# ashrafgt/k8s-gpu-hpa

Measured on AMD Instinct MI355X. Metric: p50_scrape_to_hpa_scale_latency, lower is better.
Workload: dtype bf16; 1 GPU; model=mi355x-exporter + mfma-bf16-gemm load, load=gemm_bf16 4096^3 duty-cycled, hpa=target 5, min 1, max 8 (reference rule semantics), parallelism=replicas1, gpus_exported=0, final_replicas=8, tick_aligned_steps=30, stale_steps=0

## Files before the change

### __graft_entry__.py

```python

import subprocess
import sys
from pathlib import Path

ROOT = Path(__file__).resolve().parent


def build() -> None:
    subprocess.run(
        ["make", "-C", str(ROOT / "native"), "all", "-j4",
         f"PYTHON={sys.executable}"],
        check=True,
    )
    sys.path.insert(0, str(ROOT))
    import mi355x_gpu_hpa
    import mi355x_gpu_hpa.loadgen as lg

    assert lg.available(), "libmi355x_loadgen.so missing after build"
    from mi355x_gpu_hpa.control import scraper

    assert scraper.native_available(), "libmi355x_scrape.so missing after build"
    from mi355x_gpu_hpa.control import promql

    assert promql.native_available(), (
        "_mi355x_promql extension missing after build (needs Python.h)")


def smoke() -> None:
    sys.path.insert(0, str(ROOT))
    import numpy as np
    import torch

    from mi355x_gpu_hpa import loadgen as lg

    assert torch.cuda.is_available(), "smoke() needs a GPU"
    assert lg.device_count() >= 1, lg.LoadgenError("no HIP device visible")

    rng = np.random.default_rng(0)
    a = rng.standard_normal(4096, dtype=np.float32)
    b = rng.standard_normal(4096, dtype=np.float32)
    np.testing.assert_array_equal(lg.vector_add(a, b), a + b)

    m, n, k = 128, 128, 64
    A = rng.uniform(-1, 1, (m, k)).astype(np.float32)
    Bt = rng.uniform(-1, 1, (n, k)).astype(np.float32)
    got = lg.gemm_bf16(A, Bt)
    ref = (
        torch.from_numpy(A).bfloat16().float()
        @ torch.from_numpy(Bt).bfloat16().float().T
    ).numpy()
    np.testing.assert_allclose(got, ref, rtol=2e-2, atol=1e-2)

    m, n, k = 256, 256, 128
    A = rng.uniform(-1, 1, (m, k)).astype(np.float32)
    Bt = rng.uniform(-1, 1, (n, k)).astype(np.float32)
    c, aq, btq = lg.gemm_fp8(A, Bt)
    ref8 = (aq.astype(np.float64) @ btq.astype(np.float64).T).astype(np.float32)
    np.testing.assert_allclose(c, ref8, rtol=2e-3, atol=2e-3 * np.sqrt(k))

    m, n, k = 256, 256, 256
    A = rng.uniform(-1, 1, (m, k)).astype(np.float32)
    Bt = rng.uniform(-1, 1, (n, k)).astype(np.float32)
    c, aq, btq = lg.gemm_mxfp4(A, Bt)
    ref4 = aq.astype(np.float64) @ btq.astype(np.float64).T
    np.testing.assert_allclose(
        c, ref4, rtol=2e-3,
        atol=2e-3 * np.sqrt(k) * np.abs(aq).max() * np.abs(btq).max())

    from mi355x_gpu_hpa.exporter import native_exporter_smoke

    native_exporter_smoke()
    print("smoke OK: vectorAdd + bf16/fp8/mxfp4 MFMA GEMM numerics + exporter sample")
```

### mi355x_gpu_hpa/control/__init__.py

```python
from .adapter import Adapter, AdapterError, DiscoveredMetric, discover
from .hpa import (
    HpaSpec,
    HpaState,
    MetricTarget,
    desired_replicas,
    desired_replicas_multi,
    reconcile,
    reconcile_multi,
)
from .loop import (
    REFERENCE_RULE_EXPR,
    REFERENCE_RULE_NAME,
    ControlLoop,
    LoopResult,
    RecordingRule,
    synth_pod_labels,
)
from .promql import PromQLError, Sample, evaluate, evaluate_scalar
from .scraper import Scraper, ScrapeTarget, parse_prometheus_text

__all__ = [
    "Adapter", "AdapterError", "DiscoveredMetric", "discover",
    "HpaSpec", "HpaState", "MetricTarget", "desired_replicas",
    "desired_replicas_multi", "reconcile", "reconcile_multi",
    "ControlLoop", "LoopResult", "RecordingRule", "synth_pod_labels",
    "REFERENCE_RULE_EXPR", "REFERENCE_RULE_NAME",
    "PromQLError", "Sample", "evaluate", "evaluate_scalar",
    "Scraper", "ScrapeTarget", "parse_prometheus_text",
]
```

### mi355x_gpu_hpa/control/adapter.py

```python

from __future__ import annotations

import re
from dataclasses import dataclass, field
from typing import Dict, List, Optional, Set, Tuple

from .promql import PromQLError, Sample, evaluate

RESOURCE_LABELS: Dict[str, Tuple[str, str, str]] = {
    "namespace": ("namespaces", "", "Namespace"),
    "pod": ("pods", "", "Pod"),
    "node": ("nodes", "", "Node"),
    "service": ("services", "", "Service"),
    "deployment": ("deployments", "apps", "Deployment"),
    "statefulset": ("statefulsets", "apps", "StatefulSet"),
    "daemonset": ("daemonsets", "apps", "DaemonSet"),
    "replicaset": ("replicasets", "apps", "ReplicaSet"),
    "job": ("jobs", "batch", "Job"),
    "ingress": ("ingresses", "networking.k8s.io", "Ingress"),
}

_PLURAL_TO_SINGULAR = {v[0]: k for k, v in RESOURCE_LABELS.items()}


class AdapterError(ValueError):
    pass


@dataclass
class DiscoveredMetric:

    metric: str
    series: str
    is_counter: bool
    resources: Set[str] = field(default_factory=set)


def _discoverable(s: Sample) -> bool:
    if not s.name or s.name.startswith("container_"):
        return False
    return bool(s.labels.get("namespace"))


def _metric_name(series: str) -> Tuple[str, bool]:
    m = re.match(r"^(.*)_seconds_total$", series)
    if m:
        return m.group(1), True
    m = re.match(r"^(.*)_total$", series)
    if m:
        return m.group(1), True
    return series, False


def discover(samples: List[Sample]) -> Dict[str, DiscoveredMetric]:
    out: Dict[str, DiscoveredMetric] = {}
    for s in samples:
        if not _discoverable(s):
            continue
        metric, is_counter = _metric_name(s.name)
        d = out.get(metric)
        if d is None:
            d = DiscoveredMetric(metric=metric, series=s.name,
                                 is_counter=is_counter)
            out[metric] = d
        for label, value in s.labels.items():
            if value and label in RESOURCE_LABELS:
                d.resources.add(label)
    return out


class Adapter:

    def __init__(self, samples: Optional[List[Sample]] = None):
        self._samples: List[Sample] = list(samples or [])

    def update(self, samples: List[Sample]) -> None:
        self._samples = list(samples)


    def api_resource_list(self) -> dict:
        resources = []
        for d in sorted(discover(self._samples).values(),
                        key=lambda d: d.metric):
            for label in sorted(d.resources):
                plural, group, _kind = RESOURCE_LABELS[label]
                qualified = plural if not group else f"{plural}.{group}"
                resources.append({
                    "name": f"{qualified}/{d.metric}",
                    "singularName": "",
                    "namespaced": label != "namespace",
                    "kind": "MetricValueList",
                    "verbs": ["get"],
                })
        return {
            "kind": "APIResourceList",
            "apiVersion": "v1",
            "groupVersion": "custom.metrics.k8s.io/v1beta1",
            "resources": resources,
        }

    def metric_names(self) -> Set[str]:
        return {r["name"] for r in self.api_resource_list()["resources"]}


    def get_object_metric(self, namespace: str, resource: str,
                          object_name: str, metric: str) -> dict:
        singular = _PLURAL_TO_SINGULAR.get(resource)
        if singular is None:
            raise AdapterError(f"unknown resource {resource!r}")
        for val in (namespace, object_name):
            if not re.fullmatch(r"[A-Za-z0-9._-]{1,253}", val or ""):
                raise AdapterError(f"invalid object name {val!r}")
        discovered = discover(self._samples)
        d = discovered.get(metric)
        if d is None or singular not in d.resources:
            raise AdapterError(
                f"metric {metric!r} not served for resource {resource!r}")
        if d.is_counter:
            raise AdapterError(
                f"metric {metric!r} uses a rate() query; an instant store "
                "has no range data (counters are out of this stack's path)")
        expr = (f'sum({d.series}{{namespace="{namespace}",'
                f'{singular}="{object_name}"}}) by ({singular})')
        try:
            vec = evaluate(expr, self._samples)
        except PromQLError as e:
            raise AdapterError(f"query failed: {e}") from e
        if not vec:
            raise AdapterError(
                f"no samples for {metric!r} on {resource}/{object_name} "
                f"in namespace {namespace!r}")
        plural, group, kind = RESOURCE_LABELS[singular]
        api_version = f"{group}/v1" if group else "v1"
        return {
            "kind": "MetricValueList",
            "apiVersion": "custom.metrics.k8s.io/v1beta1",
            "items": [{
                "describedObject": {
                    "kind": kind,
                    "namespace": namespace,
                    "name": object_name,
                    "apiVersion": api_version,
                },
                "metricName": metric,
                "value": vec[0].value,
            }],
        }

    def get_object_metric_value(self, namespace: str, resource: str,
                                object_name: str, metric: str
                                ) -> Optional[float]:
        try:
            resp = self.get_object_metric(namespace, resource,
                                          object_name, metric)
        except AdapterError:
            return None
        return float(resp["items"][0]["value"])
```

### mi355x_gpu_hpa/control/hpa.py

```python

from __future__ import annotations

import math
from dataclasses import dataclass, field
from typing import List, Optional, Tuple


@dataclass
class HpaSpec:
    min_replicas: int = 1
    max_replicas: int = 3
    target_value: float = 5.0
    tolerance: float = 0.1
    downscale_stabilization_s: float = 300.0
    scale_up_pods: int = 0
    scale_up_period_s: float = 15.0
    scale_down_pods: int = 0
    scale_down_period_s: float = 15.0


@dataclass
class HpaState:
    current_replicas: int = 1
    recommendations: List[Tuple[float, int]] = field(default_factory=list)
    scaleup_window: Tuple[Optional[float], Optional[int]] = (None, None)
    scaledown_window: Tuple[Optional[float], Optional[int]] = (None, None)


def desired_replicas(
    spec: HpaSpec, current_replicas: int, metric_value: Optional[float]
) -> int:
    clamp = lambda r: max(spec.min_replicas, min(spec.max_replicas, r))
    if metric_value is None:
        return clamp(current_replicas)
    if spec.target_value <= 0:
        raise ValueError("target_value must be positive")
    ratio = metric_value / spec.target_value
    if abs(ratio - 1.0) <= spec.tolerance:
        return clamp(current_replicas)
    return clamp(math.ceil(ratio * current_replicas))


@dataclass
class MetricTarget:

    name: str
    target_value: float


def desired_replicas_multi(
    spec: HpaSpec,
    metrics: List[MetricTarget],
    current_replicas: int,
    values: dict,
) -> int:
    desired = spec.min_replicas
    any_value = False
    for m in metrics:
        v = values.get(m.name)
        if v is None:
            d = current_replicas
        else:
            any_value = True
            one = HpaSpec(
                min_replicas=spec.min_replicas,
                max_replicas=spec.max_replicas,
                target_value=m.target_value,
                tolerance=spec.tolerance,
            )
            d = desired_replicas(one, current_replicas, v)
        desired = max(desired, d)
    if not any_value:
        return current_replicas
    return desired


def reconcile(
    spec: HpaSpec, state: HpaState, metric_value: Optional[float], now_s: float
) -> int:
    desired = desired_replicas(spec, state.current_replicas, metric_value)
    return _stabilize(spec, state, desired, now_s)


def reconcile_multi(
    spec: HpaSpec, state: HpaState, metrics: List[MetricTarget],
    values: dict, now_s: float
) -> int:
    desired = desired_replicas_multi(spec, metrics, state.current_replicas, values)
    return _stabilize(spec, state, desired, now_s)


def _stabilize(spec: HpaSpec, state: HpaState, desired: int, now_s: float) -> int:
    state.recommendations.append((now_s, desired))
    cutoff = now_s - spec.downscale_stabilization_s
    state.recommendations = [(t, d) for (t, d) in state.recommendations if t >= cutoff]

    stabilized = max(d for (_, d) in state.recommendations)
    new = stabilized
    if spec.scale_up_pods > 0 and new > state.current_replicas:
        base_t, base_r = state.scaleup_window
        if base_t is None or now_s - base_t >= spec.scale_up_period_s:
            base_t, base_r = now_s, state.current_replicas
        new = min(new, base_r + spec.scale_up_pods)
        state.scaleup_window = (base_t, base_r)
    if spec.scale_down_pods > 0 and new < state.current_replicas:
        base_t, base_r = state.scaledown_window
        if base_t is None or now_s - base_t >= spec.scale_down_period_s:
            base_t, base_r = now_s, state.current_replicas
        new = max(new, base_r - spec.scale_down_pods)
        state.scaledown_window = (base_t, base_r)
    new = max(spec.min_replicas, min(spec.max_replicas, new))
    state.current_replicas = new
    return new
```

### mi355x_gpu_hpa/control/scraper.py

```python

from __future__ import annotations

import ctypes
import os
import re
import time
import urllib.parse
import urllib.request
from array import array
from dataclasses import dataclass
from typing import Dict, List, Optional

from .. import NATIVE_BUILD
from .promql import Sample

SCRAPE_LIB = NATIVE_BUILD / "libmi355x_scrape.so"
NATIVE_ENV = "MI355X_SCRAPE_NATIVE"

_LINE_RE = re.compile(
    r"^(?P<name>[a-zA-Z_:][a-zA-Z0-9_:]*)"
    r"(?:\{(?P<labels>[^}]*)\})?\s+"
    r"(?P<value>[+-]?(?:\d+\.?\d*(?:[eE][+-]?\d+)?|Inf|NaN))"
    r"(?:\s+(?P<ts>-?\d+))?$"
)
_LABEL_RE = re.compile(r'([a-zA-Z_][a-zA-Z0-9_]*)="((?:[^"\\]|\\.)*)"')


def parse_prometheus_text(text: str) -> List[Sample]:
    out: List[Sample] = []
    for line in text.splitlines():
        line = line.strip()
        if not line or line.startswith("#"):
            continue
        m = _LINE_RE.match(line)
        if not m:
            continue
        labels = {}
        if m.group("labels"):
            for lm in _LABEL_RE.finditer(m.group("labels")):
                labels[lm.group(1)] = lm.group(2).replace('\\"', '"').replace(
                    "\\\\", "\\"
                )
        v = m.group("value")
        value = float("inf") if v == "Inf" else float("nan") if v == "NaN" else float(v)
        out.append(Sample(m.group("name"), labels, value))
    return out



_OK, _DEFER, _ERR_UNSUPPORTED = 0, 1, -5


class _Result(ctypes.Structure):
    _fields_ = [
        ("n_samples", ctypes.c_int32),
        ("n_strings", ctypes.c_int32),
        ("arena_len", ctypes.c_int32),
        ("body_len", ctypes.c_int32),
        ("http_status", ctypes.c_int32),
        ("connects", ctypes.c_int32),
        ("values", ctypes.c_void_p),
        ("label_counts", ctypes.c_void_p),
        ("arena", ctypes.c_void_p),
        ("body", ctypes.c_void_p),
    ]


_lib = None
_lib_tried = False


def _load_native():
    global _lib, _lib_tried
    if not _lib_tried:
        _lib_tried = True
        try:
            lib = ctypes.CDLL(str(SCRAPE_LIB))
        except OSError:
            return None
        lib.mi355x_scrape_open.restype = ctypes.c_void_p
        lib.mi355x_scrape_open.argtypes = [
            ctypes.c_char_p, ctypes.c_int, ctypes.c_char_p, ctypes.c_char_p,
            ctypes.c_double]
        lib.mi355x_scrape_close.restype = None
        lib.mi355x_scrape_close.argtypes = [ctypes.c_void_p]
        lib.mi355x_scrape_fetch.argtypes = [
            ctypes.c_void_p, ctypes.POINTER(_Result)]
        lib.mi355x_scrape_parse.argtypes = [
            ctypes.c_void_p, ctypes.c_char_p, ctypes.c_int,
            ctypes.POINTER(_Result)]
        _lib = lib
    return _lib


def native_available() -> bool:
    return _load_native() is not None


def _native_enabled_by_env() -> bool:
    return os.environ.get(NATIVE_ENV, "1").strip().lower() not in (
        "0", "false", "off", "no")


def _samples_from_result(res: _Result) -> List[Sample]:
    n = res.n_samples
    if n == 0:
        return []
    strs = ctypes.string_at(res.arena, res.arena_len).decode().split("\n")
    if len(strs) != res.n_strings + 1:
        raise ValueError("scrape library returned an inconsistent arena")
    counts = array("i")
    counts.frombytes(ctypes.string_at(res.label_counts, 4 * n))
    values = array("d")
    values.frombytes(ctypes.string_at(res.values, 8 * n))
    out: List[Sample] = []
    i = 0
    for k, v in zip(counts, values):
        j = i + 1 + 2 * k
        out.append(Sample(strs[i],
                          dict(zip(strs[i + 1:j:2], strs[i + 2:j:2])), v))
        i = j
    return out


class NativeScrapeError(OSError):

    def __init__(self, code: int, http_status: int = 0):
        super().__init__(f"native scrape failed: code {code}"
                         + (f", HTTP {http_status}" if http_status else ""))
        self.code = code
        self.http_status = http_status


class NativeClient:

    def __init__(self, host: str, port: int, path: str = "/metrics",
                 host_header: str = "", timeout_s: float = 2.0):
        lib = _load_native()
        if lib is None:
            raise OSError(f"{SCRAPE_LIB} missing; run `make -C native exporter`")
        self._lib = lib
        self._res = _Result()
        self._h = lib.mi355x_scrape_open(
            host.encode(), port, path.encode(), host_header.encode(),
            float(timeout_s))
        if not self._h:
            raise ValueError(f"bad scrape target {host!r}:{port}")

    @property
    def connects(self) -> int:
        return self._res.connects

    def _finish(self, rc: int) -> List[Sample]:
        res = self._res
        if rc == _OK:
            return _samples_from_result(res)
        if rc == _DEFER:
            return parse_prometheus_text(
                ctypes.string_at(res.body, res.body_len).decode())
        raise NativeScrapeError(rc, res.http_status)

    def fetch(self) -> List[Sample]:
        return self._finish(
            self._lib.mi355x_scrape_fetch(self._h, ctypes.byref(self._res)))

    def parse(self, data: bytes) -> List[Sample]:
        return self._finish(self._lib.mi355x_scrape_parse(
            self._h, data, len(data), ctypes.byref(self._res)))

    def close(self) -> None:
        if self._h:
            self._lib.mi355x_scrape_close(self._h)
            self._h = None

    def __del__(self):
        try:
            self.close()
        except Exception:
            pass


_parse_client: Optional[NativeClient] = None


def native_parse_prometheus_text(text: str) -> List[Sample]:
    global _parse_client
    if _parse_client is None:
        _parse_client = NativeClient("127.0.0.1", 1)
    return _parse_client.parse(text.encode())


def _native_target(url: str):
    try:
        u = urllib.parse.urlsplit(url)
        port = u.port
    except ValueError:
        return None
    if u.scheme != "http" or not u.hostname or u.username or u.password \
            or u.fragment:
        return None
    path = (u.path or "/") + ("?" + u.query if u.query else "")
    if any(c <= " " or c > "~" for c in path + u.netloc):
        return None
    return u.hostname, port or 80, path, u.netloc


@dataclass
class ScrapeTarget:
    url: str
    node: str = "node0"
    extra_labels: Optional[Dict[str, str]] = None


class Scraper:

    def __init__(self, targets: List[ScrapeTarget], timeout_s: float = 2.0,
                 native: Optional[bool] = None):
        self.targets = targets
        self.timeout_s = timeout_s
        self.last: Dict[str, List[Sample]] = {}
        self.last_scrape_duration_s: float = 0.0
        if native is None:
            native = _native_enabled_by_env()
        self.native = bool(native) and native_available()
        self._clients: Dict[str, Optional[tuple]] = {}

    def _client(self, url: str) -> Optional[NativeClient]:
        entry = self._clients.get(url, False)
        if entry and entry[0] != self.timeout_s:
            entry[1].close()
            entry = False
        if entry is False:
            spec = _native_target(url)
            entry = None
            if spec is not None:
                host, port, path, host_header = spec
                entry = (self.timeout_s, NativeClient(
                    host, port, path, host_header, self.timeout_s))
            self._clients[url] = entry
        return entry[1] if entry else None

    def _fetch_python(self, url: str) -> List[Sample]:
        with urllib.request.urlopen(url, timeout=self.timeout_s) as r:
            text = r.read().decode()
        return parse_prometheus_text(text)

    def _fetch(self, url: str) -> List[Sample]:
        client = self._client(url) if self.native else None
        if client is None:
            return self._fetch_python(url)
        try:
            return client.fetch()
        except NativeScrapeError as e:
            if e.code != _ERR_UNSUPPORTED:
                raise
            client.close()
            self._clients[url] = None
            return self._fetch_python(url)

    def close(self) -> None:
        for entry in self._clients.values():
            if entry:
                entry[1].close()
        self._clients.clear()

    def scrape_once(self) -> List[Sample]:
        t0 = time.monotonic()
        merged: List[Sample] = []
        for t in self.targets:
            try:
                samples = self._fetch(t.url)
            except Exception:
                merged.extend(self.last.get(t.url, []))
                continue
            for s in samples:
                s.labels.setdefault("node", t.node)
                if t.extra_labels:
                    for k, v in t.extra_labels.items():
                        s.labels.setdefault(k, v)
            self.last[t.url] = samples
            merged.extend(samples)
        self.last_scrape_duration_s = time.monotonic() - t0
        return merged
```

Baseline: 92.14 us.

## Move scrape relabelling, object-metric lookup and HPA reconcile into a native extension

Adds a C++ Python extension that handles the per-cycle control path natively: HTTP scrape plus parse with node and extra-label relabelling, the adapter's object-metric lookup through the native PromQL evaluator, and the HPA desired-replica and stabilization logic. Each Python entry point tries the native path first and falls back to the Python code when the extension returns DEFER. The goal is to cut Python interpreter and object-churn overhead on each scrape-to-scale cycle. In exchange there is a lot of duplicated logic that must match the Python semantics exactly, along with a string cache whose contents are cleared once it fills.

Result: faster. 58.63 us, median of 6 (-36.4%).

```diff
diff --git a/__graft_entry__.py b/__graft_entry__.py
--- a/__graft_entry__.py
+++ b/__graft_entry__.py
@@ -24,6 +24,10 @@
 
     assert promql.native_available(), (
         "_mi355x_promql extension missing after build (needs Python.h)")
+    from mi355x_gpu_hpa.control import native_cycle
+
+    assert native_cycle.native_cycle_available(), (
+        "_mi355x_control extension missing after build (needs Python.h)")
 
 
 def smoke() -> None:
diff --git a/mi355x_gpu_hpa/control/__init__.py b/mi355x_gpu_hpa/control/__init__.py
--- a/mi355x_gpu_hpa/control/__init__.py
+++ b/mi355x_gpu_hpa/control/__init__.py
@@ -16,6 +16,11 @@
     RecordingRule,
     synth_pod_labels,
 )
+from .native_cycle import (
+    native_cycle_active,
+    native_cycle_counters,
+    use_native_cycle,
+)
 from .promql import PromQLError, Sample, evaluate, evaluate_scalar
 from .scraper import Scraper, ScrapeTarget, parse_prometheus_text
 
@@ -25,6 +30,7 @@
     "desired_replicas_multi", "reconcile", "reconcile_multi",
     "ControlLoop", "LoopResult", "RecordingRule", "synth_pod_labels",
     "REFERENCE_RULE_EXPR", "REFERENCE_RULE_NAME",
+    "native_cycle_active", "native_cycle_counters", "use_native_cycle",
     "PromQLError", "Sample", "evaluate", "evaluate_scalar",
     "Scraper", "ScrapeTarget", "parse_prometheus_text",
 ]
diff --git a/mi355x_gpu_hpa/control/adapter.py b/mi355x_gpu_hpa/control/adapter.py
--- a/mi355x_gpu_hpa/control/adapter.py
+++ b/mi355x_gpu_hpa/control/adapter.py
@@ -5,6 +5,8 @@
 from dataclasses import dataclass, field
 from typing import Dict, List, Optional, Set, Tuple
 
+from . import native_cycle as _nc
+from . import promql as _promql
 from .promql import PromQLError, Sample, evaluate
 
 RESOURCE_LABELS: Dict[str, Tuple[str, str, str]] = {
@@ -150,6 +152,15 @@
     def get_object_metric_value(self, namespace: str, resource: str,
                                 object_name: str, metric: str
                                 ) -> Optional[float]:
+        if not _nc.decided:
+            _nc.use_native_cycle(None)
+        native = _nc.object_metric_value
+        native_eval = _promql._native_eval
+        if native is not None and native_eval is not None:
+            res = native(native_eval, _promql._native_defer, self._samples,
+                         namespace, resource, object_name, metric)
+            if res is not _nc.DEFER:
+                return res
         try:
             resp = self.get_object_metric(namespace, resource,
                                           object_name, metric)
diff --git a/mi355x_gpu_hpa/control/hpa.py b/mi355x_gpu_hpa/control/hpa.py
--- a/mi355x_gpu_hpa/control/hpa.py
+++ b/mi355x_gpu_hpa/control/hpa.py
@@ -4,6 +4,8 @@
 import math
 from dataclasses import dataclass, field
 from typing import List, Optional, Tuple
+
+from . import native_cycle as _nc
 
 
 @dataclass
@@ -78,6 +80,13 @@
 def reconcile(
     spec: HpaSpec, state: HpaState, metric_value: Optional[float], now_s: float
 ) -> int:
+    if not _nc.decided:
+        _nc.use_native_cycle(None)
+    native = _nc.reconcile
+    if native is not None:
+        res = native(spec, state, metric_value, now_s)
+        if res is not _nc.DEFER:
+            return res
     desired = desired_replicas(spec, state.current_replicas, metric_value)
     return _stabilize(spec, state, desired, now_s)
 
@@ -87,6 +96,13 @@
     values: dict, now_s: float
 ) -> int:
     desired = desired_replicas_multi(spec, metrics, state.current_replicas, values)
+    if not _nc.decided:
+        _nc.use_native_cycle(None)
+    native = _nc.stabilize
+    if native is not None:
+        res = native(spec, state, desired, now_s)
+        if res is not _nc.DEFER:
+            return res
     return _stabilize(spec, state, desired, now_s)
 
 
diff --git a/mi355x_gpu_hpa/control/native_cycle.py b/mi355x_gpu_hpa/control/native_cycle.py
--- /dev/null
+++ b/mi355x_gpu_hpa/control/native_cycle.py
@@ -0,0 +1,89 @@
+
+from __future__ import annotations
+
+import importlib.machinery
+import importlib.util
+import os
+from typing import Dict, Optional
+
+from .. import NATIVE_BUILD
+
+NATIVE_ENV = "MI355X_CONTROL_NATIVE"
+NATIVE_EXT_NAME = "_mi355x_control"
+
+_ext = None
+DEFER = None
+UNDECODABLE = None
+
+decided = False
+reconcile = None
+stabilize = None
+object_metric_value = None
+client_type = None
+
+
+def _ext_path():
+    return NATIVE_BUILD / (NATIVE_EXT_NAME
+                           + importlib.machinery.EXTENSION_SUFFIXES[0])
+
+
+def _load_ext():
+    global _ext, DEFER, UNDECODABLE
+    if _ext is None:
+        path = _ext_path()
+        if not path.is_file():
+            return None
+        spec = importlib.util.spec_from_file_location(
+            NATIVE_EXT_NAME, str(path))
+        try:
+            mod = importlib.util.module_from_spec(spec)
+            spec.loader.exec_module(mod)
+        except ImportError:
+            return None
+        from .hpa import HpaSpec, HpaState
+        from .promql import Sample
+        mod.bind(Sample, HpaSpec, HpaState)
+        DEFER = mod.DEFER
+        UNDECODABLE = mod.UNDECODABLE
+        _ext = mod
+    return _ext
+
+
+def native_cycle_available() -> bool:
+    return _load_ext() is not None
+
+
+def _enabled_by_env() -> bool:
+    return os.environ.get(NATIVE_ENV, "1").strip().lower() not in (
+        "0", "false", "off", "no")
+
+
+def use_native_cycle(flag: Optional[bool] = None) -> bool:
+    global decided, reconcile, stabilize, object_metric_value, client_type
+    if flag is None:
+        flag = _enabled_by_env()
+    ext = _load_ext() if flag else None
+    reconcile = ext.reconcile if ext is not None else None
+    stabilize = ext.stabilize if ext is not None else None
+    object_metric_value = (ext.object_metric_value
+                           if ext is not None else None)
+    client_type = ext.Client if ext is not None else None
+    decided = True
+    return ext is not None
+
+
+def native_cycle_active() -> bool:
+    if not decided:
+        use_native_cycle(None)
+    return reconcile is not None
+
+
+def native_cycle_counters() -> Optional[Dict[str, int]]:
+    ext = _load_ext()
+    return ext.counters() if ext is not None else None
+
+
+def reset_native_cycle_counters() -> None:
+    ext = _load_ext()
+    if ext is not None:
+        ext.reset()
diff --git a/mi355x_gpu_hpa/control/scraper.py b/mi355x_gpu_hpa/control/scraper.py
--- a/mi355x_gpu_hpa/control/scraper.py
+++ b/mi355x_gpu_hpa/control/scraper.py
@@ -12,6 +12,7 @@
 from typing import Dict, List, Optional
 
 from .. import NATIVE_BUILD
+from . import native_cycle as _nc
 from .promql import Sample
 
 SCRAPE_LIB = NATIVE_BUILD / "libmi355x_scrape.so"
@@ -141,6 +142,18 @@
             raise OSError(f"{SCRAPE_LIB} missing; run `make -C native exporter`")
         self._lib = lib
         self._res = _Result()
+        self._h = None
+        self._ext = None
+        if not _nc.decided:
+            _nc.use_native_cycle(None)
+        if _nc.client_type is not None:
+            try:
+                self._ext = _nc.client_type(host, port, path, host_header,
+                                            float(timeout_s))
+            except ValueError:
+                raise ValueError(
+                    f"bad scrape target {host!r}:{port}") from None
+            return
         self._h = lib.mi355x_scrape_open(
             host.encode(), port, path.encode(), host_header.encode(),
             float(timeout_s))
@@ -149,6 +162,8 @@
 
     @property
     def connects(self) -> int:
+        if self._ext is not None:
+            return self._ext.connects
         return self._res.connects
 
     def _finish(self, rc: int) -> List[Sample]:
@@ -160,15 +175,51 @@
                 ctypes.string_at(res.body, res.body_len).decode())
         raise NativeScrapeError(rc, res.http_status)
 
+    @staticmethod
+    def _finish_ext(res) -> List[Sample]:
+        rc, http_status, data = res
+        if rc == _DEFER:
+            return parse_prometheus_text(data.decode())
+        if rc == _nc.UNDECODABLE:
+            data.decode()
+            raise ValueError("scrape library returned an inconsistent arena")
+        raise NativeScrapeError(rc, http_status)
+
     def fetch(self) -> List[Sample]:
+        if self._ext is not None:
+            res = self._ext.fetch(None, None)
+            return res if type(res) is list else self._finish_ext(res)
         return self._finish(
             self._lib.mi355x_scrape_fetch(self._h, ctypes.byref(self._res)))
 
     def parse(self, data: bytes) -> List[Sample]:
+        if self._ext is not None:
+            res = self._ext.parse(bytes(data), None, None)
+            return res if type(res) is list else self._finish_ext(res)
         return self._finish(self._lib.mi355x_scrape_parse(
             self._h, data, len(data), ctypes.byref(self._res)))
 
+    def fetch_relabelled(self, node, extra_labels):
+        if self._ext is not None:
+            res = self._ext.fetch(node, extra_labels or None)
+            if type(res) is list:
+                return res, True
+            if res is not _nc.DEFER:
+                return self._finish_ext(res), False
+        return self.fetch(), False
+
+    def parse_relabelled(self, data: bytes, node, extra_labels):
+        if self._ext is not None:
+            res = self._ext.parse(bytes(data), node, extra_labels or None)
+            if type(res) is list:
+                return res, True
+            if res is not _nc.DEFER:
+                return self._finish_ext(res), False
+        return self.parse(data), False
+
     def close(self) -> None:
+        if self._ext is not None:
+            self._ext.close()
         if self._h:
             self._lib.mi355x_scrape_close(self._h)
             self._h = None
@@ -245,18 +296,19 @@
             text = r.read().decode()
         return parse_prometheus_text(text)
 
-    def _fetch(self, url: str) -> List[Sample]:
+    def _fetch(self, t: ScrapeTarget):
+        url = t.url
         client = self._client(url) if self.native else None
         if client is None:
-            return self._fetch_python(url)
+            return self._fetch_python(url), False
         try:
-            return client.fetch()
+            return client.fetch_relabelled(t.node, t.extra_labels)
         except NativeScrapeError as e:
             if e.code != _ERR_UNSUPPORTED:
                 raise
             client.close()
             self._clients[url] = None
-            return self._fetch_python(url)
+            return self._fetch_python(url), False
 
     def close(self) -> None:
         for entry in self._clients.values():
@@ -269,15 +321,16 @@
         merged: List[Sample] = []
         for t in self.targets:
             try:
-                samples = self._fetch(t.url)
+                samples, relabelled = self._fetch(t)
             except Exception:
                 merged.extend(self.last.get(t.url, []))
                 continue
-            for s in samples:
-                s.labels.setdefault("node", t.node)
-                if t.extra_labels:
-                    for k, v in t.extra_labels.items():
-                        s.labels.setdefault(k, v)
+            if not relabelled:
+                for s in samples:
+                    s.labels.setdefault("node", t.node)
+                    if t.extra_labels:
+                        for k, v in t.extra_labels.items():
+                            s.labels.setdefault(k, v)
             self.last[t.url] = samples
             merged.extend(samples)
         self.last_scrape_duration_s = time.monotonic() - t0
diff --git a/native/control/control_core.h b/native/control/control_core.h
--- /dev/null
+++ b/native/control/control_core.h
@@ -0,0 +1,191 @@
+#pragma once
+
+#include <cmath>
+#include <cstddef>
+#include <cstring>
+#include <limits>
+#include <memory>
+#include <string>
+#include <string_view>
+#include <unordered_map>
+#include <vector>
+
+namespace control {
+
+
+template <class V, class Release>
+class StrCache {
+ public:
+  StrCache(size_t capacity, size_t max_key, Release release)
+      : capacity_(capacity), max_key_(max_key), release_(release) {}
+  ~StrCache() { clear(); }
+  StrCache(const StrCache&) = delete;
+  StrCache& operator=(const StrCache&) = delete;
+
+  const V* find(std::string_view key) const {
+    auto it = map_.find(key);
+    return it == map_.end() ? nullptr : &it->second->value;
+  }
+
+  bool insert(std::string_view key, V value) {
+    if (key.size() > max_key_ || capacity_ == 0) return false;
+    if (map_.find(key) != map_.end()) return false;
+    if (slots_.size() >= capacity_) clear();
+    auto slot = std::make_unique<Slot>();
+    slot->key.assign(key.data(), key.size());
+    slot->value = value;
+    map_.emplace(std::string_view(slot->key), slot.get());
+    slots_.push_back(std::move(slot));
+    return true;
+  }
+
+  void clear() {
+    map_.clear();
+    for (auto& s : slots_) release_(s->value);
+    slots_.clear();
+  }
+
+  size_t size() const { return slots_.size(); }
+  size_t capacity() const { return capacity_; }
+
+ private:
+  struct Slot {
+    std::string key;
+    V value;
+  };
+  size_t capacity_;
+  size_t max_key_;
+  Release release_;
+  std::vector<std::unique_ptr<Slot>> slots_;
+  std::unordered_map<std::string_view, Slot*> map_;
+};
+
+
+inline bool valid_object_name(const char* s, size_t n) {
+  if (n < 1 || n > 253) return false;
+  for (size_t i = 0; i < n; ++i) {
+    const unsigned char c = static_cast<unsigned char>(s[i]);
+    const bool ok = (c >= 'A' && c <= 'Z') || (c >= 'a' && c <= 'z') ||
+                    (c >= '0' && c <= '9') || c == '.' || c == '_' || c == '-';
+    if (!ok) return false;
+  }
+  return true;
+}
+
+inline bool ends_with(std::string_view s, std::string_view suffix) {
+  return s.size() >= suffix.size() &&
+         std::memcmp(s.data() + s.size() - suffix.size(), suffix.data(),
+                     suffix.size()) == 0;
+}
+
+inline bool mangle_series(std::string_view series, std::string_view* metric,
+                          bool* is_counter) {
+  if (series.find('\n') != std::string_view::npos) return false;
+  static constexpr std::string_view kSeconds = "_seconds_total";
+  static constexpr std::string_view kTotal = "_total";
+  if (ends_with(series, kSeconds)) {
+    *metric = series.substr(0, series.size() - kSeconds.size());
+    *is_counter = true;
+  } else if (ends_with(series, kTotal)) {
+    *metric = series.substr(0, series.size() - kTotal.size());
+    *is_counter = true;
+  } else {
+    *metric = series;
+    *is_counter = false;
+  }
+  return true;
+}
+
+struct Resource {
+  std::string_view singular;
+  std::string_view plural;
+};
+
+constexpr Resource kResources[] = {
+    {"namespace", "namespaces"},     {"pod", "pods"},
+    {"node", "nodes"},               {"service", "services"},
+    {"deployment", "deployments"},   {"statefulset", "statefulsets"},
+    {"daemonset", "daemonsets"},     {"replicaset", "replicasets"},
+    {"job", "jobs"},                 {"ingress", "ingresses"},
+};
+constexpr int kNumResources = sizeof(kResources) / sizeof(kResources[0]);
+
+inline int resource_by_plural(std::string_view plural) {
+  for (int i = 0; i < kNumResources; ++i)
+    if (kResources[i].plural == plural) return i;
+  return -1;
+}
+
+inline int resource_by_singular(std::string_view singular) {
+  for (int i = 0; i < kNumResources; ++i)
+    if (kResources[i].singular == singular) return i;
+  return -1;
+}
+
+inline bool discoverable_name(std::string_view name) {
+  static constexpr std::string_view kContainer = "container_";
+  return !name.empty() && !(name.size() >= kContainer.size() &&
+                            name.substr(0, kContainer.size()) == kContainer);
+}
+
+
+constexpr long long kMaxExactInt = 1LL << 52;
+
+inline bool int_is_exact_time(long long v) {
+  return v >= -kMaxExactInt && v <= kMaxExactInt;
+}
+
+inline long long clamp_replicas(long long lo, long long hi, long long r) {
+  const long long m = hi < r ? hi : r;
+  return lo > m ? lo : m;
+}
+
+inline bool desired_replicas(long long min_r, long long max_r, double target,
+                             double tolerance, long long current,
+                             bool has_metric, double metric, long long* out) {
+  if (!has_metric) {
+    *out = clamp_replicas(min_r, max_r, current);
+    return true;
+  }
+  if (!(target > 0)) {
+    return false;
+  }
+  const double ratio = metric / target;
+  if (std::fabs(ratio - 1.0) <= tolerance) {
+    *out = clamp_replicas(min_r, max_r, current);
+    return true;
+  }
+  if (!int_is_exact_time(current)) return false;
+  const double product = ratio * static_cast<double>(current);
+  if (!std::isfinite(product)) return false;
+  const double c = std::ceil(product);
+  long long r;
+  if (c >= 9223372036854775808.0)
+    r = std::numeric_limits<long long>::max();
+  else if (c < -9223372036854775808.0)
+    r = std::numeric_limits<long long>::min();
+  else
+    r = static_cast<long long>(c);
+  *out = clamp_replicas(min_r, max_r, r);
+  return true;
+}
+
+inline bool in_window(double t, double cutoff) { return t >= cutoff; }
+
+inline bool apply_policy(int dir, long long pods, double period, double now,
+                         long long current, bool base_valid, double base_t,
+                         long long base_r, long long* value, bool* reset) {
+  *reset = !base_valid || now - base_t >= period;
+  const long long base = *reset ? current : base_r;
+  long long limit;
+  if (dir > 0) {
+    if (__builtin_add_overflow(base, pods, &limit)) return false;
+    if (limit < *value) *value = limit;
+  } else {
+    if (__builtin_sub_overflow(base, pods, &limit)) return false;
+    if (limit > *value) *value = limit;
+  }
+  return true;
+}
+
+}
diff --git a/native/control/control_ext.cpp b/native/control/control_ext.cpp
--- /dev/null
+++ b/native/control/control_ext.cpp
@@ -0,0 +1,840 @@
+#define PY_SSIZE_T_CLEAN
+#include <Python.h>
+
+#include <cstdint>
+#include <initializer_list>
+#include <new>
+#include <string>
+#include <string_view>
+#include <vector>
+
+#include "control_core.h"
+#include "scrape_client.h"
+
+namespace {
+
+constexpr size_t kStrCacheCapacity = 4096;
+constexpr size_t kStrCacheMaxKey = 256;
+constexpr int kUndecodable = 2;
+
+struct Counters {
+  unsigned long long scrape_handled = 0;
+  unsigned long long scrape_deferred = 0;
+  unsigned long long hpa_handled = 0;
+  unsigned long long hpa_deferred = 0;
+  unsigned long long adapter_handled = 0;
+  unsigned long long adapter_deferred = 0;
+  unsigned long long str_hits = 0;
+  unsigned long long str_misses = 0;
+} g_counters;
+
+Py_ssize_t g_str_cache_size = 0;
+
+PyObject* g_sample_type = nullptr;
+PyObject* g_spec_type = nullptr;
+PyObject* g_state_type = nullptr;
+PyObject* g_defer = nullptr;
+PyObject* g_str_node = nullptr;
+PyObject* g_str_namespace = nullptr;
+PyObject* g_attr_name = nullptr;
+PyObject* g_attr_labels = nullptr;
+PyObject* g_attr_value = nullptr;
+
+PyObject* g_n_current_replicas = nullptr;
+PyObject* g_n_downscale_stabilization_s = nullptr;
+PyObject* g_n_max_replicas = nullptr;
+PyObject* g_n_min_replicas = nullptr;
+PyObject* g_n_recommendations = nullptr;
+PyObject* g_n_scale_down_period_s = nullptr;
+PyObject* g_n_scale_down_pods = nullptr;
+PyObject* g_n_scale_up_period_s = nullptr;
+PyObject* g_n_scale_up_pods = nullptr;
+PyObject* g_n_scaledown_window = nullptr;
+PyObject* g_n_scaleup_window = nullptr;
+PyObject* g_n_target_value = nullptr;
+PyObject* g_n_tolerance = nullptr;
+
+PyObject* defer_result(unsigned long long* counter) {
+  PyErr_Clear();
+  ++*counter;
+  Py_INCREF(g_defer);
+  return g_defer;
+}
+
+
+struct DecRef {
+  void operator()(PyObject* o) const { Py_XDECREF(o); }
+};
+using PyStrCache = control::StrCache<PyObject*, DecRef>;
+
+struct ClientObject {
+  PyObject_HEAD
+  void* handle;
+  PyStrCache* cache;
+  int connects;
+  bool busy;
+};
+
+PyObject* cached_str(PyStrCache* cache, const char* p, size_t n) {
+  const std::string_view key(p, n);
+  if (const PyObject* const* hit = cache->find(key)) {
+    ++g_counters.str_hits;
+    PyObject* o = const_cast<PyObject*>(*hit);
+    Py_INCREF(o);
+    return o;
+  }
+  ++g_counters.str_misses;
+  PyObject* o = PyUnicode_DecodeUTF8(p, static_cast<Py_ssize_t>(n), nullptr);
+  if (!o) {
+    PyErr_Clear();
+    return nullptr;
+  }
+  if (cache->insert(key, o)) Py_INCREF(o);
+  return o;
+}
+
+inline bool set_default(PyObject* labels, PyObject* k, PyObject* v) {
+  const int has = PyDict_Contains(labels, k);
+  if (has < 0) return false;
+  return has == 1 || PyDict_SetItem(labels, k, v) == 0;
+}
+
+enum class Build { Ok, Undecodable, Error };
+
+Build build_samples(ClientObject* self, const mi355x_scrape_result& res,
+                    PyObject* node, PyObject* extra, PyObject** out) {
+  const Py_ssize_t n = res.n_samples;
+  PyObject* lst = PyList_New(n);
+  if (!lst) return Build::Error;
+  const char* p = res.arena;
+  const char* const end = res.arena + res.arena_len;
+  Build status = Build::Ok;
+
+  auto next_str = [&](PyObject** s) -> bool {
+    const char* nl = p < end
+        ? static_cast<const char*>(memchr(p, '\n', static_cast<size_t>(end - p)))
+        : nullptr;
+    if (!nl) {
+      status = Build::Undecodable;
+      return false;
+    }
+    *s = cached_str(self->cache, p, static_cast<size_t>(nl - p));
+    p = nl + 1;
+    if (!*s) {
+      status = Build::Undecodable;
+      return false;
+    }
+    return true;
+  };
+
+  for (Py_ssize_t i = 0; i < n && status == Build::Ok; ++i) {
+    PyObject* name = nullptr;
+    if (!next_str(&name)) break;
+    PyObject* labels = PyDict_New();
+    PyObject* value = PyFloat_FromDouble(res.values[i]);
+    bool ok = labels && value;
+    for (int32_t k = 0; ok && k < res.label_counts[i]; ++k) {
+      PyObject *key = nullptr, *val = nullptr;
+      if (!next_str(&key)) {
+        ok = false;
+        break;
+      }
+      if (!next_str(&val)) {
+        Py_DECREF(key);
+        ok = false;
+        break;
+      }
+      ok = PyDict_SetItem(labels, key, val) == 0;
+      Py_DECREF(key);
+      Py_DECREF(val);
+    }
+    if (ok && node) ok = set_default(labels, g_str_node, node);
+    if (ok && extra) {
+      Py_ssize_t pos = 0;
+      PyObject *k, *v;
+      while (ok && PyDict_Next(extra, &pos, &k, &v))
+        ok = set_default(labels, k, v);
+    }
+    PyObject* sample = nullptr;
+    if (ok) {
+      PyObject* args[3] = {name, labels, value};
+      sample = PyObject_Vectorcall(g_sample_type, args, 3, nullptr);
+    }
+    Py_XDECREF(name);
+    Py_XDECREF(labels);
+    Py_XDECREF(value);
+    if (!sample) {
+      if (status == Build::Ok) status = Build::Error;
+      break;
+    }
+    PyList_SET_ITEM(lst, i, sample);
+  }
+  g_str_cache_size = static_cast<Py_ssize_t>(self->cache->size());
+  if (status == Build::Ok && p != end) status = Build::Undecodable;
+  if (status != Build::Ok) {
+    Py_DECREF(lst);
+    return status;
+  }
+  *out = lst;
+  return Build::Ok;
+}
+
+bool relabel_args_ok(PyObject* node, PyObject* extra) {
+  if (node != Py_None && !PyUnicode_CheckExact(node)) return false;
+  if (extra == Py_None) return true;
+  if (!PyDict_CheckExact(extra)) return false;
+  Py_ssize_t pos = 0;
+  PyObject *k, *v;
+  while (PyDict_Next(extra, &pos, &k, &v))
+    if (!PyUnicode_CheckExact(k) || !PyUnicode_CheckExact(v)) return false;
+  return true;
+}
+
+PyObject* code_tuple(int rc, int http_status, const char* data, Py_ssize_t len) {
+  if (data) return Py_BuildValue("(iiy#)", rc, http_status, data, len);
+  return Py_BuildValue("(iiO)", rc, http_status, Py_None);
+}
+
+PyObject* finish(ClientObject* self, int rc, const mi355x_scrape_result& res,
+                 PyObject* node, PyObject* extra) {
+  self->connects = res.connects;
+  if (rc == MI355X_SCRAPE_OK) {
+    PyObject* lst = nullptr;
+    switch (build_samples(self, res, node == Py_None ? nullptr : node,
+                          extra == Py_None ? nullptr : extra, &lst)) {
+      case Build::Ok:
+        ++g_counters.scrape_handled;
+        return lst;
+      case Build::Undecodable:
+        ++g_counters.scrape_deferred;
+        return code_tuple(kUndecodable, res.http_status, res.arena,
+                          res.arena_len);
+      case Build::Error:
+        return nullptr;
+    }
+  }
+  if (rc == MI355X_SCRAPE_DEFER) {
+    ++g_counters.scrape_deferred;
+    return code_tuple(rc, res.http_status, res.body, res.body_len);
+  }
+  return code_tuple(rc, res.http_status, nullptr, 0);
+}
+
+PyObject* client_call(ClientObject* self, PyObject* data, PyObject* node,
+                      PyObject* extra) {
+  if (!g_sample_type || !relabel_args_ok(node, extra))
+    return defer_result(&g_counters.scrape_deferred);
+  if (!self->handle || self->busy)
+    return code_tuple(MI355X_SCRAPE_ERR_IO, 0, nullptr, 0);
+  mi355x_scrape_result res;
+  int rc;
+  self->busy = true;
+  void* const handle = self->handle;
+  if (data) {
+    const char* buf = PyBytes_AS_STRING(data);
+    const Py_ssize_t len = PyBytes_GET_SIZE(data);
+    if (len > INT32_MAX) {
+      self->busy = false;
+      return defer_result(&g_counters.scrape_deferred);
+    }
+    Py_BEGIN_ALLOW_THREADS
+    rc = mi355x_scrape_parse(handle, buf, static_cast<int>(len), &res);
+    Py_END_ALLOW_THREADS
+  } else {
+    Py_BEGIN_ALLOW_THREADS
+    rc = mi355x_scrape_fetch(handle, &res);
+    Py_END_ALLOW_THREADS
+  }
+  PyObject* out = finish(self, rc, res, node, extra);
+  self->busy = false;
+  return out;
+}
+
+PyObject* client_fetch(PyObject* self, PyObject* const* args, Py_ssize_t nargs) {
+  if (nargs != 2) {
+    PyErr_SetString(PyExc_TypeError, "fetch(node, extra_labels)");
+    return nullptr;
+  }
+  return client_call(reinterpret_cast<ClientObject*>(self), nullptr, args[0],
+                     args[1]);
+}
+
+PyObject* client_parse(PyObject* self, PyObject* const* args, Py_ssize_t nargs) {
+  if (nargs != 3 || !PyBytes_CheckExact(args[0])) {
+    PyErr_SetString(PyExc_TypeError, "parse(bytes, node, extra_labels)");
+    return nullptr;
+  }
+  return client_call(reinterpret_cast<ClientObject*>(self), args[0], args[1],
+                     args[2]);
+}
+
+PyObject* client_close(PyObject* self_, PyObject*) {
+  ClientObject* self = reinterpret_cast<ClientObject*>(self_);
+  if (self->handle && !self->busy) {
+    mi355x_scrape_close(self->handle);
+    self->handle = nullptr;
+  }
+  Py_RETURN_NONE;
+}
+
+PyObject* client_new(PyTypeObject* type, PyObject* args, PyObject*) {
+  const char *host, *path, *host_header;
+  int port;
+  double timeout_s;
+  if (!PyArg_ParseTuple(args, "sissd", &host, &port, &path, &host_header,
+                        &timeout_s))
+    return nullptr;
+  void* handle = mi355x_scrape_open(host, port, path, host_header, timeout_s);
+  if (!handle) {
+    PyErr_SetString(PyExc_ValueError, "bad scrape target");
+    return nullptr;
+  }
+  ClientObject* self = reinterpret_cast<ClientObject*>(type->tp_alloc(type, 0));
+  if (!self) {
+    mi355x_scrape_close(handle);
+    return nullptr;
+  }
+  self->handle = handle;
+  self->connects = 0;
+  self->busy = false;
+  self->cache = new (std::nothrow)
+      PyStrCache(kStrCacheCapacity, kStrCacheMaxKey, DecRef());
+  if (!self->cache) {
+    Py_DECREF(self);
+    return PyErr_NoMemory();
+  }
+  return reinterpret_cast<PyObject*>(self);
+}
+
+void client_dealloc(PyObject* self_) {
+  ClientObject* self = reinterpret_cast<ClientObject*>(self_);
+  if (self->handle) mi355x_scrape_close(self->handle);
+  delete self->cache;
+  PyTypeObject* type = Py_TYPE(self_);
+  type->tp_free(self_);
+  Py_DECREF(type);
+}
+
+PyObject* client_get_connects(PyObject* self, void*) {
+  return PyLong_FromLong(reinterpret_cast<ClientObject*>(self)->connects);
+}
+
+PyObject* client_get_cache_size(PyObject* self, void*) {
+  return PyLong_FromSize_t(reinterpret_cast<ClientObject*>(self)->cache->size());
+}
+
+PyMethodDef kClientMethods[] = {
+    {"fetch", reinterpret_cast<PyCFunction>(
+                  reinterpret_cast<void (*)()>(client_fetch)),
+     METH_FASTCALL, "fetch(node, extra_labels)"},
+    {"parse", reinterpret_cast<PyCFunction>(
+                  reinterpret_cast<void (*)()>(client_parse)),
+     METH_FASTCALL, "parse(bytes, node, extra_labels)"},
+    {"close", client_close, METH_NOARGS, "close the kept connection"},
+    {nullptr, nullptr, 0, nullptr},
+};
+
+PyGetSetDef kClientGetSet[] = {
+    {"connects", client_get_connects, nullptr,
+     "connections opened so far (as of the last call)", nullptr},
+    {"cache_size", client_get_cache_size, nullptr,
+     "strings this client's cache holds", nullptr},
+    {nullptr, nullptr, nullptr, nullptr, nullptr},
+};
+
+PyType_Slot kClientSlots[] = {
+    {Py_tp_doc, const_cast<char*>(
+                    "One target's kept connection, parser and str cache.")},
+    {Py_tp_new, reinterpret_cast<void*>(client_new)},
+    {Py_tp_dealloc, reinterpret_cast<void*>(client_dealloc)},
+    {Py_tp_methods, kClientMethods},
+    {Py_tp_getset, kClientGetSet},
+    {0, nullptr},
+};
+
+PyType_Spec kClientSpec = {
+    "_mi355x_control.Client", sizeof(ClientObject), 0, Py_TPFLAGS_DEFAULT,
+    kClientSlots,
+};
+
+
+struct Defer {};
+
+struct Attr {
+  PyObject* o;
+  Attr(PyObject* obj, PyObject* name) : o(PyObject_GetAttr(obj, name)) {
+    if (!o) throw Defer();
+  }
+  ~Attr() { Py_DECREF(o); }
+  Attr(const Attr&) = delete;
+  Attr& operator=(const Attr&) = delete;
+};
+
+long long exact_int(PyObject* o) {
+  if (!PyLong_CheckExact(o)) throw Defer();
+  int overflow = 0;
+  const long long v = PyLong_AsLongLongAndOverflow(o, &overflow);
+  if (overflow || (v == -1 && PyErr_Occurred())) throw Defer();
+  return v;
+}
+
+double exact_float(PyObject* o) {
+  if (!PyFloat_CheckExact(o)) throw Defer();
+  return PyFloat_AS_DOUBLE(o);
+}
+
+double exact_time(PyObject* o) {
+  if (PyFloat_CheckExact(o)) return PyFloat_AS_DOUBLE(o);
+  const long long v = exact_int(o);
+  if (!control::int_is_exact_time(v)) throw Defer();
+  return static_cast<double>(v);
+}
+
+struct Window {
+  bool valid = false;
+  double t = 0.0;
+  long long r = 0;
+  PyObject* t_obj = nullptr;
+  PyObject* r_obj = nullptr;
+};
+
+Window read_window(PyObject* tup) {
+  if (!PyTuple_CheckExact(tup) || PyTuple_GET_SIZE(tup) != 2) throw Defer();
+  Window w;
+  w.t_obj = PyTuple_GET_ITEM(tup, 0);
+  w.r_obj = PyTuple_GET_ITEM(tup, 1);
+  if (w.t_obj == Py_None) return w;
+  w.valid = true;
+  w.t = exact_time(w.t_obj);
+  w.r = exact_int(w.r_obj);
+  return w;
+}
+
+PyObject* stabilize_core(PyObject* spec, PyObject* state, long long desired,
+                         PyObject* now_obj, double now,
+                         long long min_r, long long max_r) {
+  const Attr a_window(spec, g_n_downscale_stabilization_s);
+  const Attr a_up_pods(spec, g_n_scale_up_pods);
+  const Attr a_up_period(spec, g_n_scale_up_period_s);
+  const Attr a_down_pods(spec, g_n_scale_down_pods);
+  const Attr a_down_period(spec, g_n_scale_down_period_s);
+  const double window = exact_float(a_window.o);
+  const long long up_pods = exact_int(a_up_pods.o);
+  const double up_period = exact_float(a_up_period.o);
+  const long long down_pods = exact_int(a_down_pods.o);
+  const double down_period = exact_float(a_down_period.o);
+
+  const Attr a_current(state, g_n_current_replicas);
+  const Attr a_recs(state, g_n_recommendations);
+  const Attr a_up_win(state, g_n_scaleup_window);
+  const Attr a_down_win(state, g_n_scaledown_window);
+  const long long current = exact_int(a_current.o);
+  PyObject* recs = a_recs.o;
+  if (!PyList_CheckExact(recs)) throw Defer();
+
+  const double cutoff = now - window;
+  const Py_ssize_t n = PyList_GET_SIZE(recs);
+  bool any = false;
+  long long best = 0;
+  Py_ssize_t dropped = 0;
+  for (Py_ssize_t i = 0; i < n; ++i) {
+    PyObject* e = PyList_GET_ITEM(recs, i);
+    if (!PyTuple_CheckExact(e) || PyTuple_GET_SIZE(e) != 2) throw Defer();
+    const double t = exact_time(PyTuple_GET_ITEM(e, 0));
+    const long long d = exact_int(PyTuple_GET_ITEM(e, 1));
+    if (!control::in_window(t, cutoff)) {
+      ++dropped;
+      continue;
+    }
+    if (!any || d > best) best = d;
+    any = true;
+  }
+  const bool keep_new = control::in_window(now, cutoff);
+  if (keep_new) {
+    if (!any || desired > best) best = desired;
+    any = true;
+  }
+  if (!any) throw Defer();
+
+  long long value = best;
+  bool up_applies = false, up_reset = false;
+  bool down_applies = false, down_reset = false;
+  Window up_win, down_win;
+  if (up_pods > 0 && value > current) {
+    up_applies = true;
+    up_win = read_window(a_up_win.o);
+    if (!control::apply_policy(+1, up_pods, up_period, now, current,
+                               up_win.valid, up_win.t, up_win.r, &value,
+                               &up_reset))
+      throw Defer();
+  }
+  if (down_pods > 0 && value < current) {
+    down_applies = true;
+    down_win = read_window(a_down_win.o);
+    if (!control::apply_policy(-1, down_pods, down_period, now, current,
+                               down_win.valid, down_win.t, down_win.r, &value,
+                               &down_reset))
+      throw Defer();
+  }
+  value = control::clamp_replicas(min_r, max_r, value);
+
+  struct Owned {
+    PyObject* o = nullptr;
+    ~Owned() { Py_XDECREF(o); }
+  } entry, up_tuple, down_tuple, result, desired_obj;
+  desired_obj.o = PyLong_FromLongLong(desired);
+  result.o = PyLong_FromLongLong(value);
+  if (!desired_obj.o || !result.o) throw Defer();
+  entry.o = PyTuple_Pack(2, now_obj, desired_obj.o);
+  if (!entry.o) throw Defer();
+  if (up_applies) {
+    up_tuple.o = up_reset ? PyTuple_Pack(2, now_obj, a_current.o)
+                          : PyTuple_Pack(2, up_win.t_obj, up_win.r_obj);
+    if (!up_tuple.o) throw Defer();
+  }
+  if (down_applies) {
+    down_tuple.o = down_reset ? PyTuple_Pack(2, now_obj, a_current.o)
+                              : PyTuple_Pack(2, down_win.t_obj, down_win.r_obj);
+    if (!down_tuple.o) throw Defer();
+  }
+
+  if (PyList_Append(recs, entry.o) < 0) throw Defer();
+  if (dropped > 0 || !keep_new) {
+    Py_ssize_t hi = PyList_GET_SIZE(recs);
+    while (hi > 0) {
+      PyObject* e = PyList_GET_ITEM(recs, hi - 1);
+      PyObject* t_obj = PyTuple_GET_ITEM(e, 0);
+      const double t = PyFloat_CheckExact(t_obj)
+                           ? PyFloat_AS_DOUBLE(t_obj)
+                           : static_cast<double>(PyLong_AsLongLong(t_obj));
+      if (control::in_window(t, cutoff)) {
+        --hi;
+        continue;
+      }
+      Py_ssize_t lo = hi - 1;
+      while (lo > 0) {
+        PyObject* e2 = PyList_GET_ITEM(recs, lo - 1);
+        PyObject* t2_obj = PyTuple_GET_ITEM(e2, 0);
+        const double t2 = PyFloat_CheckExact(t2_obj)
+                              ? PyFloat_AS_DOUBLE(t2_obj)
+                              : static_cast<double>(PyLong_AsLongLong(t2_obj));
+        if (control::in_window(t2, cutoff)) break;
+        --lo;
+      }
+      if (PyList_SetSlice(recs, lo, hi, nullptr) < 0) return nullptr;
+      hi = lo;
+    }
+  }
+  if (up_applies &&
+      PyObject_SetAttr(state, g_n_scaleup_window, up_tuple.o) < 0)
+    return nullptr;
+  if (down_applies &&
+      PyObject_SetAttr(state, g_n_scaledown_window, down_tuple.o) < 0)
+    return nullptr;
+  if (PyObject_SetAttr(state, g_n_current_replicas, result.o) < 0)
+    return nullptr;
+  Py_INCREF(result.o);
+  return result.o;
+}
+
+bool hpa_types_ok(PyObject* spec, PyObject* state) {
+  return g_spec_type && g_state_type &&
+         reinterpret_cast<PyObject*>(Py_TYPE(spec)) == g_spec_type &&
+         reinterpret_cast<PyObject*>(Py_TYPE(state)) == g_state_type;
+}
+
+PyObject* hpa_entry(PyObject* const* args, Py_ssize_t nargs, bool with_metric) {
+  if (nargs != 4) {
+    PyErr_SetString(PyExc_TypeError, "(spec, state, value, now_s)");
+    return nullptr;
+  }
+  PyObject* spec = args[0];
+  PyObject* state = args[1];
+  if (!hpa_types_ok(spec, state)) return defer_result(&g_counters.hpa_deferred);
+  try {
+    const double now = exact_time(args[3]);
+    const Attr a_min(spec, g_n_min_replicas);
+    const Attr a_max(spec, g_n_max_replicas);
+    const long long min_r = exact_int(a_min.o);
+    const long long max_r = exact_int(a_max.o);
+    long long desired;
+    if (with_metric) {
+      const Attr a_target(spec, g_n_target_value);
+      const Attr a_tol(spec, g_n_tolerance);
+      const Attr a_current(state, g_n_current_replicas);
+      const double target = exact_float(a_target.o);
+      const double tolerance = exact_float(a_tol.o);
+      const long long current = exact_int(a_current.o);
+      const bool has_metric = args[2] != Py_None;
+      const double metric = has_metric ? exact_float(args[2]) : 0.0;
+      if (!control::desired_replicas(min_r, max_r, target, tolerance, current,
+                                     has_metric, metric, &desired))
+        throw Defer();
+    } else {
+      desired = exact_int(args[2]);
+    }
+    PyObject* r = stabilize_core(spec, state, desired, args[3], now, min_r,
+                                 max_r);
+    if (r) ++g_counters.hpa_handled;
+    return r;
+  } catch (const Defer&) {
+    return defer_result(&g_counters.hpa_deferred);
+  } catch (const std::exception&) {
+    return defer_result(&g_counters.hpa_deferred);
+  }
+}
+
+PyObject* py_reconcile(PyObject*, PyObject* const* args, Py_ssize_t nargs) {
+  return hpa_entry(args, nargs, true);
+}
+
+PyObject* py_stabilize(PyObject*, PyObject* const* args, Py_ssize_t nargs) {
+  return hpa_entry(args, nargs, false);
+}
+
+
+std::string_view utf8_of(PyObject* s) {
+  Py_ssize_t len = 0;
+  const char* p = PyUnicode_AsUTF8AndSize(s, &len);
+  if (!p) throw Defer();
+  return std::string_view(p, static_cast<size_t>(len));
+}
+
+PyObject* object_metric_value(PyObject* const* args) {
+  PyObject* evaluate = args[0];
+  PyObject* evaluate_defer = args[1];
+  PyObject* samples = args[2];
+  PyObject* ns = args[3];
+  PyObject* resource = args[4];
+  PyObject* object_name = args[5];
+  PyObject* metric = args[6];
+  if (!g_sample_type || !PyCallable_Check(evaluate) ||
+      !PyList_CheckExact(samples) || !PyUnicode_CheckExact(resource) ||
+      !PyUnicode_CheckExact(metric))
+    throw Defer();
+  for (PyObject* v : {ns, object_name})
+    if (v != Py_None && !PyUnicode_CheckExact(v)) throw Defer();
+
+  const Py_ssize_t n = PyList_GET_SIZE(samples);
+  struct Series {
+    std::string_view name;
+    PyObject* labels;
+  };
+  std::vector<Series> series;
+  series.reserve(static_cast<size_t>(n));
+  struct Refs {
+    std::vector<PyObject*> v;
+    ~Refs() {
+      for (PyObject* o : v) Py_DECREF(o);
+    }
+    PyObject* keep(PyObject* o) {
+      if (!o) throw Defer();
+      v.push_back(o);
+      return o;
+    }
+  } refs;
+  for (Py_ssize_t i = 0; i < n; ++i) {
+    PyObject* s = PyList_GET_ITEM(samples, i);
+    if (reinterpret_cast<PyObject*>(Py_TYPE(s)) != g_sample_type) throw Defer();
+    PyObject* name = refs.keep(PyObject_GetAttr(s, g_attr_name));
+    PyObject* labels = refs.keep(PyObject_GetAttr(s, g_attr_labels));
+    PyObject* value = refs.keep(PyObject_GetAttr(s, g_attr_value));
+    if (!PyUnicode_CheckExact(name) || !PyDict_CheckExact(labels) ||
+        !PyFloat_CheckExact(value))
+      throw Defer();
+    Py_ssize_t pos = 0;
+    PyObject *k, *v;
+    while (PyDict_Next(labels, &pos, &k, &v))
+      if (!PyUnicode_CheckExact(k) || !PyUnicode_CheckExact(v)) throw Defer();
+    series.push_back({utf8_of(name), labels});
+  }
+
+  const int res_idx = control::resource_by_plural(utf8_of(resource));
+  if (res_idx < 0) return Py_None;
+  for (PyObject* v : {ns, object_name}) {
+    if (v == Py_None) return Py_None;
+    const std::string_view sv = utf8_of(v);
+    if (!control::valid_object_name(sv.data(), sv.size())) return Py_None;
+  }
+
+  const std::string_view want = utf8_of(metric);
+  std::string_view first_series;
+  bool found = false, is_counter = false;
+  unsigned resources = 0;
+  for (const Series& s : series) {
+    if (!control::discoverable_name(s.name)) continue;
+    PyObject* nsv = PyDict_GetItemWithError(s.labels, g_str_namespace);
+    if (!nsv) {
+      if (PyErr_Occurred()) throw Defer();
+      continue;
+    }
+    if (PyUnicode_GET_LENGTH(nsv) == 0) continue;
+    std::string_view mangled;
+    bool counter = false;
+    if (!control::mangle_series(s.name, &mangled, &counter)) throw Defer();
+    if (mangled != want) continue;
+    if (!found) {
+      found = true;
+      first_series = s.name;
+      is_counter = counter;
+    }
+    Py_ssize_t pos = 0;
+    PyObject *k, *v;
+    while (PyDict_Next(s.labels, &pos, &k, &v)) {
+      if (PyUnicode_GET_LENGTH(v) == 0) continue;
+      const int r = control::resource_by_singular(utf8_of(k));
+      if (r >= 0) resources |= 1u << r;
+    }
+  }
+  if (!found || !(resources & (1u << res_idx))) return Py_None;
+  if (is_counter) return Py_None;
+
+  const std::string_view singular = control::kResources[res_idx].singular;
+  std::string expr;
+  expr.reserve(64 + first_series.size());
+  expr.append("sum(").append(first_series).append("{namespace=\"")
+      .append(utf8_of(ns)).append("\",").append(singular).append("=\"")
+      .append(utf8_of(object_name)).append("\"}) by (").append(singular)
+      .append(")");
+  PyObject* expr_obj = refs.keep(PyUnicode_DecodeUTF8(
+      expr.data(), static_cast<Py_ssize_t>(expr.size()), nullptr));
+  PyObject* call_args[2] = {expr_obj, samples};
+  PyObject* vec = refs.keep(PyObject_Vectorcall(evaluate, call_args, 2, nullptr));
+  if (vec == evaluate_defer || !PyList_CheckExact(vec)) throw Defer();
+  if (PyList_GET_SIZE(vec) == 0) return Py_None;
+  PyObject* head = PyList_GET_ITEM(vec, 0);
+  if (reinterpret_cast<PyObject*>(Py_TYPE(head)) != g_sample_type) throw Defer();
+  PyObject* value = PyObject_GetAttr(head, g_attr_value);
+  if (!value) throw Defer();
+  if (!PyFloat_CheckExact(value)) {
+    Py_DECREF(value);
+    throw Defer();
+  }
+  return value;
+}
+
+PyObject* py_object_metric_value(PyObject*, PyObject* const* args,
+                                 Py_ssize_t nargs) {
+  if (nargs != 7) {
+    PyErr_SetString(PyExc_TypeError,
+                    "object_metric_value(evaluate, evaluate_defer, samples, "
+                    "namespace, resource, object_name, metric)");
+    return nullptr;
+  }
+  try {
+    PyObject* r = object_metric_value(args);
+    if (r == Py_None) Py_INCREF(r);
+    ++g_counters.adapter_handled;
+    return r;
+  } catch (const Defer&) {
+    return defer_result(&g_counters.adapter_deferred);
+  } catch (const std::exception&) {
+    return defer_result(&g_counters.adapter_deferred);
+  }
+}
+
+
+PyObject* py_bind(PyObject*, PyObject* args) {
+  PyObject *sample, *spec, *state;
+  if (!PyArg_ParseTuple(args, "OOO", &sample, &spec, &state)) return nullptr;
+  if (!PyType_Check(sample) || !PyType_Check(spec) || !PyType_Check(state)) {
+    PyErr_SetString(PyExc_TypeError, "bind(Sample, HpaSpec, HpaState)");
+    return nullptr;
+  }
+  Py_INCREF(sample);
+  Py_XSETREF(g_sample_type, sample);
+  Py_INCREF(spec);
+  Py_XSETREF(g_spec_type, spec);
+  Py_INCREF(state);
+  Py_XSETREF(g_state_type, state);
+  Py_RETURN_NONE;
+}
+
+PyObject* py_counters(PyObject*, PyObject*) {
+  return Py_BuildValue(
+      "{s:K,s:K,s:K,s:K,s:K,s:K,s:K,s:K,s:n}",
+      "scrape_handled", g_counters.scrape_handled,
+      "scrape_deferred", g_counters.scrape_deferred,
+      "hpa_handled", g_counters.hpa_handled,
+      "hpa_deferred", g_counters.hpa_deferred,
+      "adapter_handled", g_counters.adapter_handled,
+      "adapter_deferred", g_counters.adapter_deferred,
+      "str_cache_hits", g_counters.str_hits,
+      "str_cache_misses", g_counters.str_misses,
+      "str_cache_size", g_str_cache_size);
+}
+
+PyObject* py_reset(PyObject*, PyObject*) {
+  g_counters = Counters();
+  g_str_cache_size = 0;
+  Py_RETURN_NONE;
+}
+
+PyMethodDef kMethods[] = {
+    {"reconcile", reinterpret_cast<PyCFunction>(
+                      reinterpret_cast<void (*)()>(py_reconcile)),
+     METH_FASTCALL, "reconcile(spec, state, metric_value, now_s) -> int, or DEFER"},
+    {"stabilize", reinterpret_cast<PyCFunction>(
+                      reinterpret_cast<void (*)()>(py_stabilize)),
+     METH_FASTCALL, "stabilize(spec, state, desired, now_s) -> int, or DEFER"},
+    {"object_metric_value", reinterpret_cast<PyCFunction>(
+                                reinterpret_cast<void (*)()>(
+                                    py_object_metric_value)),
+     METH_FASTCALL, "-> float, None, or DEFER"},
+    {"bind", py_bind, METH_VARARGS, "bind(Sample, HpaSpec, HpaState)"},
+    {"counters", py_counters, METH_NOARGS,
+     "handled / deferred per entry point, string cache hits and size"},
+    {"reset", py_reset, METH_NOARGS, "zero the counters"},
+    {nullptr, nullptr, 0, nullptr},
+};
+
+PyModuleDef kModule = {
+    PyModuleDef_HEAD_INIT, "_mi355x_control",
+    "Native glue of the control cycle (see scraper.py, hpa.py, adapter.py).",
+    -1, kMethods, nullptr, nullptr, nullptr, nullptr,
+};
+
+}
+
+PyMODINIT_FUNC PyInit__mi355x_control(void) {
+  PyObject* client_type = PyType_FromSpec(&kClientSpec);
+  if (!client_type) return nullptr;
+
+  PyObject* m = PyModule_Create(&kModule);
+  if (!m) return nullptr;
+  g_defer = PyObject_CallNoArgs(reinterpret_cast<PyObject*>(&PyBaseObject_Type));
+  g_str_node = PyUnicode_InternFromString("node");
+  g_str_namespace = PyUnicode_InternFromString("namespace");
+  g_attr_name = PyUnicode_InternFromString("name");
+  g_attr_labels = PyUnicode_InternFromString("labels");
+  g_attr_value = PyUnicode_InternFromString("value");
+  g_n_current_replicas = PyUnicode_InternFromString("current_replicas");
+  g_n_downscale_stabilization_s = PyUnicode_InternFromString("downscale_stabilization_s");
+  g_n_max_replicas = PyUnicode_InternFromString("max_replicas");
+  g_n_min_replicas = PyUnicode_InternFromString("min_replicas");
+  g_n_recommendations = PyUnicode_InternFromString("recommendations");
+  g_n_scale_down_period_s = PyUnicode_InternFromString("scale_down_period_s");
+  g_n_scale_down_pods = PyUnicode_InternFromString("scale_down_pods");
+  g_n_scale_up_period_s = PyUnicode_InternFromString("scale_up_period_s");
+  g_n_scale_up_pods = PyUnicode_InternFromString("scale_up_pods");
+  g_n_scaledown_window = PyUnicode_InternFromString("scaledown_window");
+  g_n_scaleup_window = PyUnicode_InternFromString("scaleup_window");
+  g_n_target_value = PyUnicode_InternFromString("target_value");
+  g_n_tolerance = PyUnicode_InternFromString("tolerance");
+  bool ok = g_n_current_replicas && g_n_downscale_stabilization_s && g_n_max_replicas && g_n_min_replicas && g_n_recommendations && g_n_scale_down_period_s && g_n_scale_down_pods && g_n_scale_up_period_s && g_n_scale_up_pods && g_n_scaledown_window && g_n_scaleup_window && g_n_target_value && g_n_tolerance &&
+            g_defer && g_str_node && g_str_namespace && g_attr_name &&
+            g_attr_labels && g_attr_value;
+  if (ok) {
+    Py_INCREF(g_defer);
+    ok = PyModule_AddObject(m, "DEFER", g_defer) == 0 &&
+         PyModule_AddObject(m, "Client", client_type) == 0 &&
+         PyModule_AddIntConstant(m, "UNDECODABLE", kUndecodable) == 0 &&
+         PyModule_AddIntConstant(m, "STR_CACHE_CAPACITY",
+                                 static_cast<long>(kStrCacheCapacity)) == 0;
+  }
+  if (!ok) {
+    Py_DECREF(m);
+    return nullptr;
+  }
+  return m;
+}
diff --git a/native/control/control_selftest.cpp b/native/control/control_selftest.cpp
--- /dev/null
+++ b/native/control/control_selftest.cpp
@@ -0,0 +1,241 @@
+#include <cmath>
+#include <cstdio>
+#include <cstdlib>
+#include <limits>
+#include <random>
+#include <string>
+
+#include "control_core.h"
+
+namespace {
+
+int g_failed = 0;
+
+#define CHECK(cond)                                                     \
+  do {                                                                  \
+    if (!(cond)) {                                                      \
+      std::fprintf(stderr, "%s:%d: CHECK failed: %s\n", __FILE__,       \
+                   __LINE__, #cond);                                    \
+      ++g_failed;                                                       \
+    }                                                                   \
+  } while (0)
+
+struct Live {
+  int count = 0;
+};
+Live g_live;
+
+struct Release {
+  void operator()(int* p) const {
+    --g_live.count;
+    delete p;
+  }
+};
+
+int* make(int v) {
+  ++g_live.count;
+  return new int(v);
+}
+
+void test_cache() {
+  using Cache = control::StrCache<int*, Release>;
+  {
+    Cache c(4, 8, Release());
+    CHECK(c.size() == 0 && c.find("a") == nullptr);
+    {
+      std::string k = "gpu";
+      CHECK(c.insert(k, make(1)));
+      k.assign("xxx");
+    }
+    CHECK(c.find("gpu") && **c.find("gpu") == 1);
+    CHECK(c.find("gp") == nullptr && c.find("gpuu") == nullptr);
+    CHECK(c.insert(std::string_view("a\0b", 3), make(2)));
+    CHECK(c.find(std::string_view("a\0b", 3)) &&
+          c.find(std::string_view("a\0c", 3)) == nullptr &&
+          c.find("a") == nullptr);
+    CHECK(c.insert("", make(3)) && **c.find("") == 3);
+    int* dup = make(9);
+    CHECK(!c.insert("gpu", dup));
+    Release()(dup);
+    int* big = make(9);
+    CHECK(!c.insert("123456789", big) && c.find("123456789") == nullptr);
+    Release()(big);
+    CHECK(c.insert("12345678", make(4)) && c.size() == 4);
+    CHECK(g_live.count == 4);
+    CHECK(c.insert("new", make(5)));
+    CHECK(c.size() == 1 && g_live.count == 1);
+    CHECK(c.find("gpu") == nullptr && **c.find("new") == 5);
+  }
+  CHECK(g_live.count == 0);
+
+  {
+    Cache zero(0, 8, Release());
+    int* v = make(1);
+    CHECK(!zero.insert("a", v));
+    Release()(v);
+  }
+
+  {
+    Cache c(64, 32, Release());
+    std::mt19937 rng(7);
+    for (int i = 0; i < 20000; ++i) {
+      const int k = static_cast<int>(rng() % 500);
+      const std::string key = "pod-" + std::to_string(k);
+      if (const int* const* hit = c.find(key)) {
+        CHECK(**hit == k);
+      } else {
+        CHECK(c.insert(key, make(k)));
+      }
+      CHECK(c.size() <= 64 && static_cast<int>(c.size()) == g_live.count);
+    }
+  }
+  CHECK(g_live.count == 0);
+}
+
+void test_names() {
+  auto valid = [](const std::string& s) {
+    return control::valid_object_name(s.data(), s.size());
+  };
+  CHECK(valid("cuda-test") && valid("a") && valid("A.b_c-9"));
+  CHECK(!valid("") && !valid("a b") && !valid("a\"") && !valid("a\\") &&
+        !valid("a\n") && !valid("caf\xc3\xa9") && !valid(std::string("a\0b", 3)));
+  CHECK(valid(std::string(253, 'x')) && !valid(std::string(254, 'x')));
+
+  auto mangle = [](const std::string& s, std::string* m, bool* c) {
+    std::string_view v;
+    const bool ok = control::mangle_series(s, &v, c);
+    if (ok) m->assign(v);
+    return ok;
+  };
+  std::string m;
+  bool c = false;
+  CHECK(mangle("cuda_test_gpu_avg", &m, &c) && m == "cuda_test_gpu_avg" && !c);
+  CHECK(mangle("http_requests_total", &m, &c) && m == "http_requests" && c);
+  CHECK(mangle("cpu_seconds_total", &m, &c) && m == "cpu" && c);
+  CHECK(mangle("_seconds_total", &m, &c) && m.empty() && c);
+  CHECK(mangle("_total", &m, &c) && m.empty() && c);
+  CHECK(mangle("total", &m, &c) && m == "total" && !c);
+  CHECK(mangle("x_total_", &m, &c) && m == "x_total_" && !c);
+  CHECK(mangle("", &m, &c) && m.empty() && !c);
+  CHECK(!mangle("a\n_total", &m, &c) && !mangle("a_total\n", &m, &c));
+
+  CHECK(control::discoverable_name("dcgm_gpu_utilization"));
+  CHECK(!control::discoverable_name("") &&
+        !control::discoverable_name("container_cpu") &&
+        !control::discoverable_name("container_"));
+  CHECK(control::discoverable_name("container") &&
+        control::discoverable_name("xcontainer_"));
+
+  CHECK(control::kNumResources == 10);
+  for (int i = 0; i < control::kNumResources; ++i) {
+    CHECK(control::resource_by_plural(control::kResources[i].plural) == i);
+    CHECK(control::resource_by_singular(control::kResources[i].singular) == i);
+  }
+  CHECK(control::resource_by_plural("deployment") == -1 &&
+        control::resource_by_plural("") == -1 &&
+        control::resource_by_singular("deployments") == -1);
+  CHECK(control::resource_by_plural("ingresses") ==
+        control::resource_by_singular("ingress"));
+}
+
+void test_replicas() {
+  const double nan = std::numeric_limits<double>::quiet_NaN();
+  const double inf = std::numeric_limits<double>::infinity();
+  const long long llmax = std::numeric_limits<long long>::max();
+  const long long llmin = std::numeric_limits<long long>::min();
+
+  CHECK(control::clamp_replicas(1, 8, 0) == 1 &&
+        control::clamp_replicas(1, 8, 9) == 8 &&
+        control::clamp_replicas(1, 8, 5) == 5);
+  CHECK(control::clamp_replicas(5, 3, 4) == 5 &&
+        control::clamp_replicas(5, 3, 1) == 5);
+  CHECK(control::clamp_replicas(llmin, llmax, llmax) == llmax);
+
+  long long d = 0;
+  CHECK(control::desired_replicas(1, 8, 0.0, 0.1, 12, false, 0.0, &d) && d == 8);
+  CHECK(control::desired_replicas(1, 8, 40.0, 0.1, 1, true, 80.0, &d) && d == 2);
+  CHECK(control::desired_replicas(1, 8, 40.0, 0.1, 4, true, 81.7, &d) && d == 8);
+  CHECK(control::desired_replicas(1, 8, 40.0, 0.1, 3, true, 43.9, &d) && d == 3);
+  CHECK(control::desired_replicas(1, 8, 40.0, 0.1, 3, true, 44.1, &d) && d == 4);
+  CHECK(control::desired_replicas(-9, 8, 5.0, 0.1, 3, true, -1.0, &d) && d == 0);
+  CHECK(control::desired_replicas(1, 8, 5.0, 0.1, 3, true, 0.0, &d) && d == 1);
+  CHECK(!control::desired_replicas(1, 8, 0.0, 0.1, 3, true, 1.0, &d));
+  CHECK(!control::desired_replicas(1, 8, -1.0, 0.1, 3, true, 1.0, &d));
+  CHECK(!control::desired_replicas(1, 8, nan, 0.1, 3, true, 1.0, &d));
+  CHECK(!control::desired_replicas(1, 8, 5.0, 0.1, 3, true, nan, &d));
+  CHECK(!control::desired_replicas(1, 8, 5.0, 0.1, 3, true, inf, &d));
+  CHECK(!control::desired_replicas(1, 8, 5.0, 0.1, 3, true, -inf, &d));
+  CHECK(!control::desired_replicas(1, 8, 5.0, 0.1, 0, true, inf, &d));
+  CHECK(control::desired_replicas(1, 8, 5.0, 0.1, 3, true, 1e308, &d) && d == 8);
+  CHECK(control::desired_replicas(1, 8, 5.0, 0.1, 3, true, -1e308, &d) && d == 1);
+  CHECK(control::desired_replicas(llmin, llmax, 5.0, 0.1, 3, true, 1e308, &d) &&
+        d == llmax);
+  CHECK(control::desired_replicas(llmin, llmax, 5.0, 0.1, 3, true, -1e308, &d) &&
+        d == llmin);
+  CHECK(control::desired_replicas(7, 2, 5.0, 0.1, 3, true, 1e308, &d) && d == 7);
+  CHECK(!control::desired_replicas(1, 8, 1e-300, 0.1, 3, true, 1e10, &d));
+  CHECK(!control::desired_replicas(1, 8, 5.0, 0.1, llmax, true, 7.0, &d));
+  CHECK(control::desired_replicas(1, 8, 5.0, inf, 3, true, inf, &d) && d == 3);
+  CHECK(control::desired_replicas(1, 8, 5.0, nan, 3, true, 5.0, &d) && d == 3);
+  CHECK(control::desired_replicas(llmin, llmax, 1.0, 0.0, 1LL << 40, true,
+                                  1048576.0, &d) && d == (1LL << 60));
+  CHECK(control::desired_replicas(llmin, llmax, 1.0, 0.0, 1LL << 40, true,
+                                  4194304.0, &d) && d == (1LL << 62));
+  CHECK(control::desired_replicas(llmin, llmax, 1.0, 0.0, 1LL << 40, true,
+                                  8388608.0, &d) && d == llmax);
+
+  CHECK(control::int_is_exact_time(0) &&
+        control::int_is_exact_time(control::kMaxExactInt) &&
+        control::int_is_exact_time(-control::kMaxExactInt) &&
+        !control::int_is_exact_time(control::kMaxExactInt + 1) &&
+        !control::int_is_exact_time(llmin));
+
+  CHECK(control::in_window(700.0, 1000.0 - 300.0) &&
+        !control::in_window(699.9, 1000.0 - 300.0));
+  CHECK(!control::in_window(5.0, nan) && !control::in_window(nan, 5.0));
+  CHECK(control::in_window(inf, inf - 300.0));
+
+  long long v = 8;
+  bool reset = false;
+  CHECK(control::apply_policy(+1, 2, 15.0, 100.0, 1, false, 0.0, 0, &v,
+                              &reset) && reset && v == 3);
+  v = 8;
+  CHECK(control::apply_policy(+1, 2, 15.0, 110.0, 3, true, 100.0, 1, &v,
+                              &reset) && !reset && v == 3);
+  v = 8;
+  CHECK(control::apply_policy(+1, 2, 15.0, 115.0, 3, true, 100.0, 1, &v,
+                              &reset) && reset && v == 5);
+  v = 4;
+  CHECK(control::apply_policy(+1, 4, 15.0, 101.0, 3, true, 100.0, 1, &v,
+                              &reset) && !reset && v == 4);
+  v = 1;
+  CHECK(control::apply_policy(-1, 1, 15.0, 100.0, 8, false, 0.0, 0, &v,
+                              &reset) && reset && v == 7);
+  v = 1;
+  CHECK(control::apply_policy(-1, 1, 15.0, 105.0, 7, true, 100.0, 8, &v,
+                              &reset) && !reset && v == 7);
+  v = 8;
+  CHECK(control::apply_policy(+1, 2, nan, 1e9, 3, true, 100.0, 1, &v,
+                              &reset) && !reset && v == 3);
+  v = 8;
+  CHECK(!control::apply_policy(+1, llmax, 15.0, 100.0, 1, false, 0.0, 0, &v,
+                               &reset));
+  CHECK(!control::apply_policy(-1, llmax, 15.0, 100.0, -2, false, 0.0, 0, &v,
+                               &reset));
+  CHECK(!control::apply_policy(+1, 1, 15.0, 101.0, 3, true, 100.0, llmax, &v,
+                               &reset));
+}
+
+}
+
+int main() {
+  test_cache();
+  test_names();
+  test_replicas();
+  if (g_failed) {
+    std::fprintf(stderr, "control-selftest: %d check(s) failed\n", g_failed);
+    return 1;
+  }
+  std::puts("control-selftest: ok");
+  return 0;
+}
```
